# jabberjabberjabber/video-3d-pipeline

Measured on AMD Instinct MI355X. Metric: 1080p_sbs_to_4k_depth_frames_per_s, higher is better.
Workload: dtype int16 (SGM) + f64 (guided filter sums; f32 depth in/out)

## Files before the change

### video-3d-pipeline_amd/csrc/v3d_guided.hip

```cpp
#include "v3d_common.h"
#include <type_traits>

__device__ __forceinline__ double gf_rcp(double x)
{
    double r = __builtin_amdgcn_rcp(x);
    r = fma(r, fma(-x, r, 1.0), r);
    r = fma(r, fma(-x, r, 1.0), r);
    return r;
}

template <typename TD> __device__ __forceinline__ float gf_ld(const TD* p, size_t i);
template <> __device__ __forceinline__ float gf_ld<float>(const float* p, size_t i) { const float v = p[i]; return fabsf(v) <= 3.402823466e38f ? v : 0.f; }
template <> __device__ __forceinline__ float gf_ld<int16_t>(const int16_t* p, size_t i) { const int d = p[i]; return d > 0 ? (float)d * 0.0625f : 0.f; }
template <> __device__ __forceinline__ float gf_ld<uint16_t>(const uint16_t* p, size_t i) { return (float)p[i]; }

typedef unsigned short v3d_u16x2v __attribute__((ext_vector_type(2)));
typedef unsigned short v3d_u16x4 __attribute__((ext_vector_type(4)));
__device__ __forceinline__ void gf_st(float* p, float q) { *p = q; }
__device__ __forceinline__ void gf_st(uint16_t* p, float q) { *p = v3d_rint_u16(q); }

#define GF_TX 64
#define GF_RUN 8
#define GF_RMAX 16

template <typename TD>
__device__ __forceinline__ double gf_bilinear(const TD* __restrict__ src, int Ws, int Hs, double sx, double sy, int x, int y)
{
    const double fx = (x + 0.5) * sx - 0.5, fy = (y + 0.5) * sy - 0.5;
    const double x0f = floor(fx), y0f = floor(fy);
    const double wx = fx - x0f, wy = fy - y0f;
    const int x0 = (int)x0f, y0 = (int)y0f;
    const int xa = min(max(x0, 0), Ws - 1), xb = min(max(x0 + 1, 0), Ws - 1);
    const int ya = min(max(y0, 0), Hs - 1), yb = min(max(y0 + 1, 0), Hs - 1);
    const double top = (double)gf_ld(src, (size_t)ya * Ws + xa) * (1.0 - wx) + (double)gf_ld(src, (size_t)ya * Ws + xb) * wx;
    const double bot = (double)gf_ld(src, (size_t)yb * Ws + xa) * (1.0 - wx) + (double)gf_ld(src, (size_t)yb * Ws + xb) * wx;
    return top * (1.0 - wy) + bot * wy;
}

template <int SWEEP, int GF_RUNY, typename TD, typename TO>
__global__ __launch_bounds__(256) void k_gf(const TD* __restrict__ depth_lo, int Wlo, int Hlo,
                                            const uint8_t* __restrict__ guide, int W, int H, int r, double eps,
                                            double* __restrict__ A, double* __restrict__ B, TO* __restrict__ out)
{
    constexpr int NS = SWEEP == 1 ? 4 : 2;
    constexpr int GF_TY = 4 * GF_RUNY;
    extern __shared__ __attribute__((aligned(16))) double smem[];
    const int rows = GF_TY + 2 * r;
    const int pitch = (GF_TX + 2 * r) | 1;
    const int hp = GF_TX + 1;
    double* t0 = smem;
    double* t1 = t0 + rows * pitch;
    double* hs = t1 + rows * pitch;

// ... 230 lines not shown
                                asm volatile("" : "+v"(cg), "+v"(cgg) :: "memory");
                            }
                        }
                        const double s0a = cq[0] + fq[0], s0b = cq[0] + lq[0], s1a = cq[1] + fq[1], s1b = cq[1] + lq[1];
                        const int cy = min(y + RR, H - 1) - max(y - RR, 0) + 1;
                        const int cx0 = min(hgx + RR, W - 1) - max(hgx - RR, 0) + 1, cx1 = min(hgx + 1 + RR, W - 1) - max(hgx + 1 - RR, 0) + 1;
                        const double inva = gf_rcp((double)(cx0 * cy)), invb = cx1 == cx0 ? inva : gf_rcp((double)(cx1 * cy));
                        const size_t o = (size_t)y * W + hgx;
                        if (SWEEP == 1) {
                            const int sga = cg + g0, sgb = cg + gl, sgga = cgg + gg0, sggb = cgg + ggl;
                            double ab[2][2];
#pragma unroll
                            for (int n = 0; n < 2; n++) {
                                const double inv = n ? invb : inva;
                                const double mI = (double)(n ? sgb : sga) * (inv * (1.0 / 255.0)), mp = (n ? s0b : s0a) * inv;
                                const double mII = (double)(n ? sggb : sgga) * (inv * (1.0 / 65025.0)), mIp = (n ? s1b : s1a) * (inv * (1.0 / 255.0));
                                const double var = fma(-mI, mI, mII), cov = fma(-mI, mp, mIp);
                                const double a = cov * gf_rcp(var + eps);
                                ab[n][0] = a; ab[n][1] = fma(-a, mI, mp);
                            }
                            if (vec_ok) {
                                v3d_f64x2 va = { ab[0][0], ab[1][0] }, vb = { ab[0][1], ab[1][1] };
                                __builtin_nontemporal_store(va, reinterpret_cast<v3d_f64x2*>(A + o));
                                __builtin_nontemporal_store(vb, reinterpret_cast<v3d_f64x2*>(B + o));
                            } else {
                                A[o] = ab[0][0]; B[o] = ab[0][1];
                                if (px1) { A[o + 1] = ab[1][0]; B[o + 1] = ab[1][1]; }
                            }
                        } else {
                            const double Ia = (double)guide[o] * (1.0 / 255.0);
                            const double Ib = px1 ? (double)guide[o + 1] * (1.0 / 255.0) : 0.0;
                            const float qa = (float)((s0a * inva) * Ia + (s1a * inva)), qb = (float)((s0b * invb) * Ib + (s1b * invb));
                            if (vec_ok && (std::is_same<TO, float>::value || (reinterpret_cast<uintptr_t>(out + o) & 3) == 0)) {
                                if constexpr (std::is_same<TO, float>::value) {
                                    v3d_f32x2 vq = { qa, qb };
                                    __builtin_nontemporal_store(vq, reinterpret_cast<v3d_f32x2*>(out + o));
                                } else {
                                    v3d_u16x2v vq = { v3d_rint_u16(qa), v3d_rint_u16(qb) };
                                    __builtin_nontemporal_store(vq, reinterpret_cast<v3d_u16x2v*>(out + o));
                                }
                            } else {
                                gf_st(out + o, qa);
                                if (px1) gf_st(out + o + 1, qb);
                            }
                        }
                    }
                    buf ^= 1;
                }
            }
        }
    }
}

__device__ __forceinline__ int gf_swz2(int m) { return m ^ ((m >> 3) & 1) ^ ((m >> 4) & 1); }
__device__ __forceinline__ int gf_swz4(int m) { return m ^ ((m >> 4) & 3); }
__device__ __forceinline__ int gf_c8(int c) { return 2 * gf_swz2(c >> 1) + (c & 1); }

template <int RR>
__device__ __forceinline__ void gf_run4(const double* row, int c0, double s[4])
{
    const v3d_f64x2* d = reinterpret_cast<const v3d_f64x2*>(row);
    const int m0 = (c0 - RR) >> 1;
    double c = 0.0, l0 = 0.0, l1 = 0.0, l2 = 0.0, r1 = 0.0, r2 = 0.0, r3 = 0.0;
#pragma unroll
    for (int k0 = 0; k0 < RR + 2; k0 += GF_CH) {
        v3d_f64x2 w[GF_CH];
#pragma unroll
        for (int i = 0; i < GF_CH; i++) if (k0 + i < RR + 2) w[i] = d[gf_swz2(m0 + k0 + i)];
#pragma unroll
        for (int i = 0; i < GF_CH; i++) {
            const int k = k0 + i;
            if (k == 0) { l0 = w[i].x; l1 = w[i].y; c = w[i].x; c += w[i].y; }
            else if (k == 1) { l2 = w[i].x; c += w[i].x; c += w[i].y; }
            else if (k < RR) { c += w[i].x; c += w[i].y; }
            else if (k == RR) { c += w[i].x; r1 = w[i].y; }
            else if (k == RR + 1) { r2 = w[i].x; r3 = w[i].y; }
        }
        asm volatile("" : "+v"(c) :: "memory");
    }
    s[0] = c; s[1] = (s[0] + r1) - l0; s[2] = (s[1] + r2) - l1; s[3] = (s[2] + r3) - l2;
}

template <int RR>
__device__ __forceinline__ void gf_run4(const int2* row, int c0, int2 s[4])
{
    const int4* d = reinterpret_cast<const int4*>(row);
    const int m0 = (c0 - RR) >> 1;
    int2 c = make_int2(0, 0), l0 = c, l1 = c, l2 = c, r1 = c, r2 = c, r3 = c;
#pragma unroll
    for (int k0 = 0; k0 < RR + 2; k0 += 3) {
        int4 w[3];
#pragma unroll
        for (int i = 0; i < 3; i++) if (k0 + i < RR + 2) w[i] = d[gf_swz2(m0 + k0 + i)];
#pragma unroll
        for (int i = 0; i < 3; i++) {
            const int k = k0 + i;
            const int2 a = make_int2(w[i].x, w[i].y), b = make_int2(w[i].z, w[i].w);
            if (k == 0) { l0 = a; l1 = b; c = make_int2(a.x + b.x, a.y + b.y); }
            else if (k == 1) { l2 = a; c.x += a.x + b.x; c.y += a.y + b.y; }
            else if (k < RR) { c.x += a.x + b.x; c.y += a.y + b.y; }
            else if (k == RR) { c.x += a.x; c.y += a.y; r1 = b; }
            else if (k == RR + 1) { r2 = a; r3 = b; }
        }
        asm volatile("" : "+v"(c.x), "+v"(c.y) :: "memory");
    }
    s[0] = c;
    s[1] = make_int2(s[0].x + r1.x - l0.x, s[0].y + r1.y - l0.y);
    s[2] = make_int2(s[1].x + r2.x - l1.x, s[1].y + r2.y - l1.y);
    s[3] = make_int2(s[2].x + r3.x - l2.x, s[2].y + r3.y - l2.y);
}

template <int RR>
__device__ __forceinline__ void gf_run4(const int4* row, int c0, int4 s[4])
{
    int4 c = make_int4(0, 0, 0, 0), l0 = c, l1 = c, l2 = c, r1 = c, r2 = c, r3 = c;
#pragma unroll
    for (int k0 = 0; k0 < 2 * RR + 4; k0 += 3) {
        int4 u[3];
#pragma unroll
        for (int i = 0; i < 3; i++) if (k0 + i < 2 * RR + 4) u[i] = row[gf_swz4(c0 - RR + k0 + i)];
#pragma unroll
        for (int i = 0; i < 3; i++) {
            const int k = k0 + i;
            if (k < 2 * RR + 1) { c.x += u[i].x; c.y += u[i].y; c.z += u[i].z; c.w += u[i].w; }
            if (k == 0) l0 = u[i];
            else if (k == 1) l1 = u[i];
            else if (k == 2) l2 = u[i];
            else if (k == 2 * RR + 1) r1 = u[i];
            else if (k == 2 * RR + 2) r2 = u[i];
            else if (k == 2 * RR + 3) r3 = u[i];
        }
        asm volatile("" : "+v"(c.x), "+v"(c.y), "+v"(c.z), "+v"(c.w) :: "memory");
    }
    s[0] = c;
    s[1] = make_int4(s[0].x - l0.x + r1.x, s[0].y - l0.y + r1.y, s[0].z - l0.z + r1.z, s[0].w - l0.w + r1.w);
    s[2] = make_int4(s[1].x - l1.x + r2.x, s[1].y - l1.y + r2.y, s[1].z - l1.z + r2.z, s[1].w - l1.w + r2.w);
    s[3] = make_int4(s[2].x - l2.x + r3.x, s[2].y - l2.y + r3.y, s[2].z - l2.z + r3.z, s[2].w - l2.w + r3.w);
}

template <int RR>
__device__ __forceinline__ void gf_solve4(const int sg[4], const int sgg[4], const double sp[4], const double sgp[4], int hgx, int y,
                                          int W, int H, double eps, double a[4], double b[4])
{
    const int cy = min(y + RR, H - 1) - max(y - RR, 0) + 1;
    int cx[4];
#pragma unroll
    for (int n = 0; n < 4; n++) cx[n] = min(hgx + n + RR, W - 1) - max(hgx + n - RR, 0) + 1;
    const double inv0 = gf_rcp((double)(cx[0] * cy));
#pragma unroll
    for (int n = 0; n < 4; n++) {
        const double inv = (n == 0 || cx[n] == cx[0]) ? inv0 : gf_rcp((double)(cx[n] * cy));
        const double mI = (double)sg[n] * (inv * (1.0 / 255.0)), mp = sp[n] * inv;
        const double mII = (double)sgg[n] * (inv * (1.0 / 65025.0)), mIp = sgp[n] * (inv * (1.0 / 255.0));
        const double var = fma(-mI, mI, mII), cov = fma(-mI, mp, mIp);
        const double aa = cov * gf_rcp(var + eps);
        a[n] = aa; b[n] = fma(-aa, mI, mp);
    }
}

template <int RR, int COLS, typename TD, bool I1, typename TO>
__global__ __launch_bounds__(2 * COLS, I1 ? 4 : 2) void k_gff(const TD* __restrict__ depth_lo, int Wlo, int Hlo,
                                                const uint8_t* __restrict__ guide, int W, int H, double eps, int band_h,
                                                TO* __restrict__ out, size_t depth_stride, size_t guide_stride)
{
    static_assert(RR % 4 == 0, "runs of four must not straddle the strip's halo boundaries");
    static_assert(!I1 || std::is_same<TD, int16_t>::value, "the integer stage 1 takes the int16 disparity");
    static_assert(COLS == 256 || (COLS == 512 && I1), "strip width (512 columns: I1 only, the f64 route's rows exceed the LDS)");
    constexpr int R = 2 * RR + 1, NOUT = COLS - 4 * RR, HR = COLS / 4;
    constexpr int S1D = 2 * 4 * 2 * COLS * 8, S1 = I1 ? 2 * 4 * COLS * 16 : S1D + 2 * 4 * COLS * 8;
    __shared__ __attribute__((aligned(16))) unsigned char sS1[S1];
    double (*sV1)[4][2][COLS] = reinterpret_cast<double (*)[4][2][COLS]>(sS1);
    int2 (*sVi)[4][COLS] = reinterpret_cast<int2 (*)[4][COLS]>(sS1 + (I1 ? 0 : S1D));
    int4 (*sVq)[4][COLS] = reinterpret_cast<int4 (*)[4][COLS]>(sS1);
// ... 17 lines not shown
        const int gxc = min(max(gx, 0), W - 1);
        uint32_t ring[R];
        double r1[I1 ? 1 : R];
        uint32_t rgw[I1 ? 1 : (R + 3) / 4];
        int vg = 0, vgg = 0, vP = 0, vgP = 0;
        double v0 = 0.0, v1 = 0.0;
#pragma unroll
        for (int j = 0; j < R; j++) ring[j] = 0u;
#pragma unroll
        for (int j = 0; j < (I1 ? 1 : R); j++) r1[j] = 0.0;
#pragma unroll
        for (int j = 0; j < (I1 ? 1 : (R + 3) / 4); j++) rgw[j] = 0u;
        (void)ring; (void)r1; (void)rgw;
        int bxa, bxb, wxa = 0, wxb = 0; double bwx = 0.0;
        const double sx = (double)Wlo / (double)W, sy = (double)Hlo / (double)H;
        if constexpr (I1) {
            const int kx = gx >> 1;
            bxa = min(max((gx & 1) ? kx : kx - 1, 0), Wlo - 1); bxb = min(max((gx & 1) ? kx + 1 : kx, 0), Wlo - 1);
            wxa = (gx & 1) ? 3 : 1; wxb = 4 - wxa;
        } else {
            const double fx = (gx + 0.5) * sx - 0.5, x0f = floor(fx);
            bwx = fx - x0f;
            bxa = min(max((int)x0f, 0), Wlo - 1); bxb = min(max((int)x0f + 1, 0), Wlo - 1);
        }
        (void)wxa; (void)wxb; (void)bwx;
        struct RowIn { int g; typename std::conditional<I1, int, float>::type a0, a1, b0, b1; bool in; };
        auto fetch_row = [&](int tt) -> RowIn {
            RowIn q;
            const int e = ya - 2 * RR + tt;
            q.in = col_ok && e >= 0 && e < H && tt < nrows;
            const int ec = min(max(e, 0), H - 1);
            q.g = guide[(size_t)ec * W + gxc];
            if constexpr (I1) {
                const int ky = ec >> 1;
                const TD* ra = depth_lo + (size_t)min(max((ec & 1) ? ky : ky - 1, 0), Hlo - 1) * Wlo;
                const TD* rb = depth_lo + (size_t)min(max((ec & 1) ? ky + 1 : ky, 0), Hlo - 1) * Wlo;
                q.a0 = max((int)ra[bxa], 0); q.a1 = max((int)ra[bxb], 0); q.b0 = max((int)rb[bxa], 0); q.b1 = max((int)rb[bxb], 0);
            } else {
                const double fy = (e + 0.5) * sy - 0.5, y0f = floor(fy);
                const TD* ra = depth_lo + (size_t)min(max((int)y0f, 0), Hlo - 1) * Wlo;
                const TD* rb = depth_lo + (size_t)min(max((int)y0f + 1, 0), Hlo - 1) * Wlo;
                q.a0 = gf_ld(ra, bxa); q.a1 = gf_ld(ra, bxb); q.b0 = gf_ld(rb, bxa); q.b1 = gf_ld(rb, bxb);
            }
            return q;
        };
        RowIn nx[4] = { fetch_row(0), fetch_row(1), fetch_row(2), fetch_row(3) };
        for (int p0 = 0; p0 < NP; p0 += R) {
#pragma clang loop unroll(full)
            for (int sp = 0; sp < R; sp++) {
                const int p = p0 + sp;
                if (p < NP) {
                    int tl = t;
                    asm volatile("" : "+v"(tl));
                    const int hrow = tl / HR, c0 = 4 * (tl % HR), hgx = gx0 + c0;
                    const int j = p - 1;
                    if (j >= RR / 2 && j < NS) {
                        const int y = ya - 3 * RR + 4 * j + hrow;
                        double a[4] = { 0.0, 0.0, 0.0, 0.0 }, b[4] = { 0.0, 0.0, 0.0, 0.0 };
                        if (c0 >= RR && c0 < COLS - RR && y >= 0 && y < H && hgx >= 0 && hgx < W) {
                            int sg[4], sgg[4]; double sp_[4], sgp[4];
                            if constexpr (I1) {
                                int4 s[4];
                                gf_run4<RR>(&sVq[j & 1][hrow][0], c0, s);
#pragma unroll
                                for (int n = 0; n < 4; n++) {
                                    sg[n] = s[n].x; sgg[n] = s[n].y;
                                    sp_[n] = (double)s[n].z * (1.0 / 256.0); sgp[n] = (double)s[n].w * (1.0 / 256.0);
                                }
                            } else {
                                int2 si[4];
                                gf_run4<RR>(&sVi[j & 1][hrow][0], c0, si);
                                gf_run4<RR>(&sV1[j & 1][hrow][0][0], c0, sp_);
                                gf_run4<RR>(&sV1[j & 1][hrow][1][0], c0, sgp);
#pragma unroll
                                for (int n = 0; n < 4; n++) { sg[n] = si[n].x; sgg[n] = si[n].y; }
                            }
                            gf_solve4<RR>(sg, sgg, sp_, sgp, hgx, y, W, H, eps, a, b);
#pragma unroll
                            for (int n = 0; n < 4; n++) if (hgx + n >= W) { a[n] = 0.0; b[n] = 0.0; }
                        }
                        double* ab = &sAB[j % 3][hrow][0][0];
                        const int e0 = 2 * gf_swz2(c0 >> 1), e1 = 2 * gf_swz2((c0 >> 1) + 1);
                        *reinterpret_cast<v3d_f64x2*>(ab + e0) = v3d_f64x2{ a[0], a[1] };
                        *reinterpret_cast<v3d_f64x2*>(ab + e1) = v3d_f64x2{ a[2], a[3] };
                        *reinterpret_cast<v3d_f64x2*>(ab + COLS + e0) = v3d_f64x2{ b[0], b[1] };
                        *reinterpret_cast<v3d_f64x2*>(ab + COLS + e1) = v3d_f64x2{ b[2], b[3] };
                    }
                    if (p < NS) {
                        const int tA = 4 * p;
                        const RowIn cur[4] = { nx[0], nx[1], nx[2], nx[3] };
#pragma unroll
                        for (int k = 0; k < 4; k++) nx[k] = fetch_row(tA + 4 + k);
                        const bool emit = p >= RR / 2;
#pragma unroll
                        for (int rr = 0; rr < 4; rr++) {
                            const int slot = (4 * sp + rr) % R;
                            const int e = ya - 2 * RR + tA + rr;
                            if constexpr (I1) {
                                int gn = 0, Pn = 0;
                                if (cur[rr].in) {
                                    gn = cur[rr].g;
                                    const int wya = (e & 1) ? 3 : 1;
                                    Pn = wya * (wxa * cur[rr].a0 + wxb * cur[rr].a1) + (4 - wya) * (wxa * cur[rr].b0 + wxb * cur[rr].b1);
                                }
                                const int go = (int)(ring[slot] & 0xFFu), Po = (int)(ring[slot] >> 8);
                                ring[slot] = ((uint32_t)Pn << 8) | (uint32_t)gn;
                                vg += gn - go; vgg += gn * gn - go * go;
                                vP += Pn - Po; vgP += gn * Pn - go * Po;
                                if (emit) sVq[p & 1][rr][gf_swz4(t)] = make_int4(vg, vgg, vP, vgP);
                            } else {
                                int gn = 0; double pn = 0.0;
                                if (cur[rr].in) {
                                    gn = cur[rr].g;
                                    const double fy = (e + 0.5) * sy - 0.5, wy = fy - floor(fy);
                                    const double a0 = (double)cur[rr].a0, b0 = (double)cur[rr].b0;
                                    const double top = fma(bwx, (double)cur[rr].a1 - a0, a0);
                                    const double bot = fma(bwx, (double)cur[rr].b1 - b0, b0);
                                    pn = fma(wy, bot - top, top);
                                }
                                const int go = (int)((rgw[slot >> 2] >> (8 * (slot & 3))) & 0xFFu); const double po = r1[slot];
                                rgw[slot >> 2] = (rgw[slot >> 2] & ~(0xFFu << (8 * (slot & 3)))) | ((uint32_t)gn << (8 * (slot & 3)));
                                r1[slot] = pn;
                                vg += gn - go; vgg += gn * gn - go * go;
                                v0 += pn - po; v1 = fma((double)gn, pn, fma(-(double)go, po, v1));
                                if (emit) {
                                    const int ct = gf_c8(t);
                                    sV1[p & 1][rr][0][ct] = v0; sV1[p & 1][rr][1][ct] = v1;
                                    sVi[p & 1][rr][ct] = make_int2(vg, vgg);
                                }
                            }
                        }
                    }
                    __syncthreads();
                }
            }
        }
    } else {
        double r0[R], r1[R], va = 0.0, vb = 0.0;
#pragma unroll
        for (int j = 0; j < R; j++) { r0[j] = 0.0; r1[j] = 0.0; }
        for (int p0 = 0; p0 < NP; p0 += R) {
#pragma clang loop unroll(full)
            for (int sp = 0; sp < R; sp++) {
                const int p = p0 + sp;
                if (p < NP) {
                    int tl = t;
                    asm volatile("" : "+v"(tl));
                    const int hrow = tl / HR, c0 = 4 * (tl % HR), hgx = gx0 + c0;
                    {
                        const int j = p - 3;
                        const int y = ya - 4 * RR + 4 * j + hrow;
                        if (j >= RR && j < NS && c0 >= 2 * RR && c0 < COLS - 2 * RR && hgx < W && y < yb) {
                            double sa[4], sb[4];
                            gf_run4<RR>(&sAB[j % 3][hrow][0][0], c0, sa);
                            gf_run4<RR>(&sAB[j % 3][hrow][1][0], c0, sb);
                            const int cy = min(y + RR, H - 1) - max(y - RR, 0) + 1;
                            int cx[4];
#pragma unroll
                            for (int n = 0; n < 4; n++) cx[n] = min(hgx + n + RR, W - 1) - max(hgx + n - RR, 0) + 1;
                            const double inv0 = gf_rcp((double)(cx[0] * cy));
                            const size_t o = (size_t)y * W + hgx;
                            const bool all_in = hgx + 3 < W;
                            const bool vec_ok = all_in && (W & 3) == 0 && ((reinterpret_cast<uintptr_t>(out + o) | reinterpret_cast<uintptr_t>(guide + o)) & 3) == 0
                                                && (reinterpret_cast<uintptr_t>(out + o) & (4 * sizeof(TO) - 1)) == 0;
                            int g[4];
                            if (vec_ok) {
                                const uint32_t g4 = *reinterpret_cast<const uint32_t*>(guide + o);
#pragma unroll
                                for (int n = 0; n < 4; n++) g[n] = (g4 >> (8 * n)) & 0xFF;
                            } else {
#pragma unroll
                                for (int n = 0; n < 4; n++) g[n] = hgx + n < W ? guide[o + n] : 0;
                            }
                            float q[4];
#pragma unroll
                            for (int n = 0; n < 4; n++) {
                                const double inv = (n == 0 || cx[n] == cx[0]) ? inv0 : gf_rcp((double)(cx[n] * cy));
                                const double I = (double)g[n] * (1.0 / 255.0);
                                q[n] = (float)((sa[n] * inv) * I + (sb[n] * inv));
                            }
                            if (vec_ok) {
                                if constexpr (std::is_same<TO, float>::value) {
                                    const v3d_f32x4 vq = { q[0], q[1], q[2], q[3] };
                                    __builtin_nontemporal_store(vq, reinterpret_cast<v3d_f32x4*>(out + o));
                                } else {
                                    const v3d_u16x4 vq = { v3d_rint_u16(q[0]), v3d_rint_u16(q[1]), v3d_rint_u16(q[2]), v3d_rint_u16(q[3]) };
                                    __builtin_nontemporal_store(vq, reinterpret_cast<v3d_u16x4*>(out + o));
                                }
                            } else {
#pragma unroll
                                for (int n = 0; n < 4; n++) if (hgx + n < W) gf_st(out + o + n, q[n]);
                            }
                        }
                    }
                    {
                        const int j = p - 2;
                        if (j >= RR / 2 && j < NS) {
                            const bool emit = j >= RR;
                            double* col = &sAB[j % 3][0][0][gf_c8(tl)];
#pragma unroll
                            for (int rr = 0; rr < 4; rr++) {
                                const int slot = (4 * sp + rr) % R;
                                const double n0 = col[rr * 2 * COLS], n1 = col[rr * 2 * COLS + COLS];
                                const double o0 = r0[slot], o1 = r1[slot];
                                r0[slot] = n0; r1[slot] = n1;
                                va += n0 - o0; vb += n1 - o1;
                                if (emit) { col[rr * 2 * COLS] = va; col[rr * 2 * COLS + COLS] = vb; }
                            }
                        }
                    }
                    __syncthreads();
                }
            }
        }
    }
}

template <int RR, typename TD, typename TO>
static void launch_gff(const TD* depth_lo, int Wlo, int Hlo, const uint8_t* guide, int W, int H, double eps,
                       TO* out, int n, size_t depth_stride, size_t guide_stride, hipStream_t st)
{
    bool i1 = false;
    if constexpr (std::is_same<TD, int16_t>::value) i1 = g_v3d_opt.gf_int1 && W == 2 * Wlo && H == 2 * Hlo;
    const int cols = g_v3d_opt.gf_cols == 512 && i1 ? 512 : 256;
    int band = g_v3d_opt.gf_band;
    if (band <= 0) {
        int dev = 0, ncu = 256;
        (void)hipGetDevice(&dev);
        (void)hipDeviceGetAttribute(&ncu, hipDeviceAttributeMultiprocessorCount, dev);
        const long slots = (long)ncu * (cols == 256 && i1 ? 2 : 1), strips = v3d_cdiv(W, cols - 4 * RR);
        long best = -1;
        for (int nb = 1; nb <= 64 && nb <= H; nb++) {
            const int b = (v3d_cdiv(H, nb) + 1) & ~1;
            const long wgs = strips * v3d_cdiv(H, b) * n, rounds = (wgs + slots - 1) / slots, cost = rounds * (b + 4 * RR);
            if (best < 0 || cost < best) { best = cost; band = b; }
        }
    }
    const dim3 grid(v3d_cdiv(W, cols - 4 * RR), v3d_cdiv(H, band), n);
    if constexpr (std::is_same<TD, int16_t>::value) {
        if (i1 && cols == 512) {
            hipLaunchKernelGGL((k_gff<RR, 512, TD, true, TO>), grid, dim3(1024), 0, st, depth_lo, Wlo, Hlo, guide, W, H, eps, band, out, depth_stride, guide_stride);
            return;
        }
        if (i1) {
            hipLaunchKernelGGL((k_gff<RR, 256, TD, true, TO>), grid, dim3(512), 0, st, depth_lo, Wlo, Hlo, guide, W, H, eps, band, out, depth_stride, guide_stride);
            return;
        }
    }
    hipLaunchKernelGGL((k_gff<RR, 256, TD, false, TO>), grid, dim3(512), 0, st, depth_lo, Wlo, Hlo, guide, W, H, eps, band, out, depth_stride, guide_stride);
}

template <int RR, typename TD, typename TO>
// ... 93 lines not shown
```

### video-3d-pipeline_amd/csrc/v3d_sgbm_cost.hip

```cpp
#include "v3d_sgbm_internal.h"

#ifndef PF_BAND
#define PF_BAND 64
#endif
__global__ __launch_bounds__(256) void k_prefilter(const uint8_t* __restrict__ img1, const uint8_t* __restrict__ img2,
                                                   int W, int H, int pitch, size_t frame_stride, int ft,
                                                   uint4* __restrict__ rec)
{
    __shared__ uint8_t sI[2][2][256];
    __shared__ unsigned short sGR[2][2][256];
    const int t = threadIdx.x, f = blockIdx.z;
    const int x = blockIdx.x * 252 - 2 + t;
    const int xc = min(max(x, 0), W - 1);
    const bool xin = x > 0 && x < W - 1;
    const int ya = blockIdx.y * PF_BAND, yb = min(ya + PF_BAND, H);
    const uint8_t* I0 = img1 + f * frame_stride + xc;
    const uint8_t* I1 = img2 + f * frame_stride + xc;
    auto ld = [&](int y) -> uint32_t {
        const size_t o = (size_t)min(max(y, 0), H - 1) * pitch;
        return (uint32_t)I0[o] | ((uint32_t)I1[o] << 8);
    };
    int dm[2], d0[2], r0[2];
    {
        const uint32_t vm = ld(ya - 1), v0 = ld(ya);
// ... 8 lines not shown
            r0[im] = (v0 >> (8 * im)) & 0xFF;
        }
        __syncthreads();
    }
    uint32_t nxt = ld(ya + 1);
    int gp[2] = { 0, 0 }, rp[2] = { 0, 0 };
    const int tl = max(t - 1, 0), tr = min(t + 1, 255);
    for (int y = ya; y <= yb; y++) {
        const int par = y & 1;
        const uint32_t ve = nxt;
        nxt = ld(y + 2);
        sI[par][0][t] = (uint8_t)ve; sI[par][1][t] = (uint8_t)(ve >> 8);
        sGR[par][0][t] = (unsigned short)(gp[0] | (rp[0] << 8));
        sGR[par][1][t] = (unsigned short)(gp[1] | (rp[1] << 8));
        __syncthreads();
        uint32_t out[4];
#pragma unroll
        for (int im = 0; im < 2; im++) {
            const int g = gp[im], r = rp[im];
            const int lo = sGR[par][im][tl], hi = sGR[par][im][tr];
            int gl = g, gr = g, rl = r, rr = r;
            if (x > 0) { gl = (g + (lo & 0xFF)) >> 1; rl = (r + (lo >> 8)) >> 1; }
            if (x < W - 1) { gr = (g + (hi & 0xFF)) >> 1; rr = (r + (hi >> 8)) >> 1; }
            const int g0 = min(min(gl, gr), g), g1 = max(max(gl, gr), g);
            const int q0 = min(min(rl, rr), r), q1 = max(max(rl, rr), r);
            out[2 * im] = (uint32_t)g | ((uint32_t)g0 << 8) | ((uint32_t)g1 << 16);
            out[2 * im + 1] = (uint32_t)r | ((uint32_t)q0 << 8) | ((uint32_t)q1 << 16);
            const int de = (int)sI[par][im][tr] - (int)sI[par][im][tl];
            const int dup = y > 0 ? dm[im] : d0[im];
            const int ddn = y < H - 1 ? de : d0[im];
            gp[im] = xin ? min(max(2 * d0[im] + dup + ddn, -ft), ft) + ft : ft;
            rp[im] = xin ? r0[im] : ft;
            dm[im] = d0[im]; d0[im] = de; r0[im] = (ve >> (8 * im)) & 0xFF;
        }
        if (y > ya && t >= 2 && t <= 253 && x < W)
            st_stream(rec + ((size_t)f * H + (y - 1)) * W + x, make_uint4(out[0], out[1], out[2], out[3]));
    }
}

template <int LPC> struct CostGeo {
    static constexpr int EP = 64 / LPC, NP = EP / 2, COLS = 512 / LPC, OUT = COLS - 4, NREC = COLS + 64;
};
#ifndef V3D_COST_LPC
#define V3D_COST_LPC 8
#endif

__device__ __forceinline__ uint32_t bt_pair(uint32_t U, uint32_t U0, uint32_t U1, uint32_t V, uint32_t V0, uint32_t V1)
{
    const uint32_t a = pk_max(pk_subu_sat(U, V1), pk_subu_sat(V0, U));
    const uint32_t b = pk_max(pk_subu_sat(V, U1), pk_subu_sat(U0, V));
    return pk_min(a, b);
}

#ifndef V3D_COST_WAVES
#define V3D_COST_WAVES 6
#endif
template <int LPC>
__global__ __launch_bounds__(512, V3D_COST_WAVES) void k_cost(const uint4* __restrict__ rec,
                                              int W, int H, int W1, int lofs, int band_h, int P2, unsigned char* __restrict__ C, int xcd_order)
{
    typedef CostGeo<LPC> G;
    constexpr int EP = G::EP, NP = G::NP, COLS = G::COLS, OUT = G::OUT, NREC = G::NREC;
    typedef typename VecT<EP>::type vec_t;
    constexpr int RROW = (NREC + 4) / 2, RCOPY = 6 * RROW + (LPC == 8 ? 3 : 0), RBUF = 2 * RCOPY;
    __shared__ __attribute__((aligned(8))) uint32_t sRV[2 * RBUF];
    __shared__ __attribute__((aligned(8))) uint32_t sUL[2][COLS][6];
    __shared__ vec_t sPix[2][COLS][LPC];

    const int tid = threadIdx.x, col = tid / LPC, dq = tid % LPC;
    int bxi = blockIdx.x, byi = blockIdx.y, bzi = blockIdx.z;
    if (xcd_order) xcd_tile(bxi, byi, bzi);
    const int xr0 = bxi * OUT;
    const int ys = byi * band_h, ye = min(ys + band_h, H);
    const int f = bzi;
    const uint32_t* rf = reinterpret_cast<const uint32_t*>(rec + (size_t)f * H * W);
    unsigned char* Cf = C + (size_t)f * c_frame(H, W1);
    static_assert(LPC == 8, "the store packs a lane's 8 disparities into one 12-byte field");

    const int xrc = min(max(xr0 - 2 + col, 0), W1 - 1);
    const int k0 = NREC - 66 - (xrc - xr0) + EP * dq;
    const int rcopy = k0 & 1, rk = k0 - rcopy;
    const int rv_off = rcopy * RCOPY + rk / 2;
    const bool out_col = (col >= 2) && (col < 2 + OUT) && (xr0 - 2 + col < W1);
    const int hc = min(max(col, 2), COLS - 3);
    const int nrows = (ye - ys) + 4;

    const int half = tid & 1, ri = tid >> 1, lt = (tid - 256) >> 1;
    const bool ld_right = ri < NREC, ld_left = tid >= 256 && lt < COLS;
    uint32_t ld_a = 0, ld_b = 0;
    int st_off = 0;
    if (ld_right) {
        ld_a = 4 * min(max(xr0 - 1 + ri, 0), W - 1) + 2 + half;
        ld_b = 4 * min(max(xr0 - 2 + ri, 0), W - 1) + 2 + half;
        const int k = NREC - 1 - ri;
        st_off = (k & 1) * RCOPY + 3 * half * RROW + (k >> 1);
    } else if (ld_left) {
        ld_a = ld_b = 4 * (min(max(xr0 - 2 + lt, 0), W1 - 1) + lofs) + half;
        st_off = lt * 6 + 3 * half;
    }
    const bool ld_any = ld_right || ld_left;
    auto stage = [&](int b, uint2 rec) {
        if (ld_right) {
#pragma unroll
            for (int j = 0; j < 3; j++)
                sRV[b * RBUF + st_off + j * RROW] = __builtin_amdgcn_perm(rec.y, rec.x, 0x0c000c00u | (uint32_t)j | ((uint32_t)(4 + j) << 16));
        } else if (ld_left) {
#pragma unroll
            for (int j = 0; j < 3; j++)
                (&sUL[b][0][0])[st_off + j] = __builtin_amdgcn_perm(rec.x, rec.x, 0x0c000c00u | (uint32_t)j | ((uint32_t)j << 16));
        }
    };
    const __amdgpu_buffer_rsrc_t rs_rec = buf_rsrc(rf, (uint32_t)H * W * 16u), rs_c = buf_rsrc(Cf, (uint32_t)c_frame(H, W1));
    const uint32_t la = ld_any ? ld_a * 4u : V3D_BUF_OOB, lb = ld_any ? ld_b * 4u : V3D_BUF_OOB;
    auto fetch = [&](int k) -> uint2 {
        const uint32_t ro = (uint32_t)min(max(ys - 2 + min(k, nrows - 1), 0), H - 1) * W * 16u;
        return make_uint2(buf_load_u32(rs_rec, ro + la), buf_load_u32(rs_rec, ro + lb));
    };
    if (ld_any) stage(0, fetch(0));
    uint2 nr[2];
    nr[1] = fetch(1); nr[0] = fetch(2);
    __syncthreads();

    uint32_t ring[5][NP], vs[NP];
#pragma unroll
    for (int j = 0; j < NP; j++) { vs[j] = 0u;
#pragma unroll
        for (int i = 0; i < 5; i++) ring[i][j] = 0u; }
    const uint32_t st_col = out_col ? (uint32_t)((xr0 - 2 + col) * C_PXB + c_lane_off<EP>(dq)) : V3D_BUF_OOB;

    for (int k10 = 0; k10 < nrows; k10 += 10) {
#pragma unroll
      for (int s10 = 0; s10 < 10; s10++) {
        const int k = k10 + s10;
        if (k >= nrows) break;
        const int slot = s10 % 5, buf = s10 & 1;

        uint32_t pix[NP];
#pragma unroll
        for (int pl = 0; pl < 2; pl++) {
            uint32_t U[3], V[3][NP];
#pragma unroll
            for (int i = 0; i < 3; i++) {
                U[i] = sUL[buf][col][3 * pl + i];
                const uint32_t* pr = &sRV[buf * RBUF + rv_off + (3 * pl + i) * RROW];
#pragma unroll
                for (int j = 0; j < NP; j++) V[i][j] = pr[j];
            }
#pragma unroll
            for (int j = 0; j < NP; j++) {
                const uint32_t c = bt_pair(U[0], U[1], U[2], V[0][j], V[1][j], V[2][j]);
                pix[j] = pl == 0 ? c : pix[j] + pk_shr_u(c, 2);
            }
            if (pl == 0) { if (NP == 4) asm volatile("" : "+v"(pix[0]), "+v"(pix[1]), "+v"(pix[NP - 2]), "+v"(pix[NP - 1]) :: "memory");
                           else asm volatile("" : "+v"(pix[0]), "+v"(pix[NP - 1]) :: "memory"); }
        }
        sPix[buf][col][dq] = Packer<NP>::go(pix);

        if (k + 1 < nrows && ld_any) stage(buf ^ 1, nr[buf ^ 1]);
        nr[buf ^ 1] = fetch(k + 3);
        __syncthreads();

        {
            uint32_t h[NP], w[NP];
            vec_unpack<NP>(sPix[buf][hc - 2][dq], h);
#pragma unroll
            for (int t = -1; t <= 2; t++) {
                vec_unpack<NP>(sPix[buf][hc + t][dq], w);
#pragma unroll
                for (int j = 0; j < NP; j++) h[j] += w[j];
            }
#pragma unroll
            for (int j = 0; j < NP; j++) { vs[j] += h[j] - ring[slot][j]; ring[slot][j] = h[j]; }
            const uint32_t st_row = k >= 4 ? (uint32_t)c_row(ys + k - 4, W1) : V3D_BUF_OOB;
            const uint32_t st_off = __builtin_elementwise_add_sat(st_col, st_row);
            {
                uint32_t t[NP];
#pragma unroll
                for (int j = 0; j < NP; j++)
                    asm("v_bfi_b32 %0, %1, %2, %3" : "=v"(t[j]) : "s"(0xFFFu), "v"(vs[j]), "v"(vs[j] >> 4));
                const v3d_u32x3_a4 pk = { __builtin_amdgcn_perm(t[1], t[0], 0x04020100u), __builtin_amdgcn_perm(t[2], t[1], 0x05040201u),
                                          __builtin_amdgcn_perm(t[NP - 1], t[2], 0x06050402u) };
                __builtin_amdgcn_raw_buffer_store_b96(pk, rs_c, st_off, 0, 2);
            }
        }
      }
    }
}

__global__ __launch_bounds__(256) void k_c_export(const unsigned char* __restrict__ C, size_t npx, int P2, int16_t* __restrict__ out)
{
    const size_t i = (size_t)blockIdx.x * 256 + threadIdx.x, px = i >> 3;
    const int dl = (int)(i & 7);
    if (px >= npx) return;
    const uint4 v = c_unpack(*reinterpret_cast<const typename CRaw<8>::type*>(C + px * C_PXB + c_lane_off<8>(dl)), dl, pk_bcast(P2));
    *reinterpret_cast<uint4*>(out + px * V3D_D + 8 * dl) = v;
}

int sgbm_cost_volume(v3d_sgbm* h, const uint8_t* left, const uint8_t* right, int n, int W, int H, int pitch, size_t frame_stride, hipStream_t st)
{
    const int W1 = W - V3D_D;
    prof_mark(h, ST_PREFILTER, st);
    hipLaunchKernelGGL(k_prefilter, dim3(v3d_cdiv(W, 252), v3d_cdiv(H, PF_BAND), n), dim3(256), 0, st, left, right, W, H, pitch, frame_stride, h->ftzero, h->rec);
    prof_mark(h, ST_COST, st);
    constexpr int COST_OUT = CostGeo<V3D_COST_LPC>::OUT;
    hipLaunchKernelGGL((k_cost<V3D_COST_LPC>), dim3(v3d_cdiv(W1, COST_OUT), v3d_cdiv(H, h->cost_band), n), dim3(512), 0, st, h->rec, W, H, W1, V3D_D + h->prm.minDisparity, h->cost_band, h->P2, h->C, h->cost_xcd);
    V3D_LAUNCH_CHECK();
    return V3D_OK;
}

int sgbm_export_cost(const v3d_sgbm* h, int W, int H, int16_t* C_out, hipStream_t st)
{
    const size_t npx = (size_t)(W - V3D_D) * H;
    hipLaunchKernelGGL(k_c_export, dim3((unsigned)((npx * 8 + 255) / 256)), dim3(256), 0, st, h->C, npx, h->P2, C_out);
    V3D_LAUNCH_CHECK();
    return V3D_OK;
}
```

Measured before the change: 2588.

## Replace XOR-swizzled shared-memory layout with parity-interleaved layout in guided filter

Replaces the XOR swizzles (gf_swz2/gf_swz4/gf_c8) on the guided-filter shared-memory row buffers with a layout that splits columns by parity or by mod 4 into separate contiguous sections. Each horizontal running-sum load then becomes a per-thread base pointer plus a compile-time constant offset, which removes per-load swizzle arithmetic. The layout is meant to keep consecutive threads on distinct LDS banks. The vertical pass now indexes by the raw thread id, relying on that pass being elementwise and in place. The new layout could bring back bank conflicts if the interleave maps threads poorly, and it depends on COLS being divisible by 4.

```diff
diff --git a/video-3d-pipeline_amd/csrc/v3d_gf_layout.h b/video-3d-pipeline_amd/csrc/v3d_gf_layout.h
--- /dev/null
+++ b/video-3d-pipeline_amd/csrc/v3d_gf_layout.h
@@ -0,0 +1,16 @@
+#pragma once
+
+#if defined(__HIPCC__)
+#define GF_LAY_FN __host__ __device__ __forceinline__ constexpr
+#else
+#define GF_LAY_FN static inline
+#endif
+
+GF_LAY_FN int gf_pair_chunk(int m, int cols) { return (m & 1) * (cols / 4) + (m >> 1); }
+GF_LAY_FN int gf_pair_elem(int c, int cols) { return 2 * gf_pair_chunk(c >> 1, cols) + (c & 1); }
+GF_LAY_FN int gf_pair_col(int t, int cols) { return t < cols / 2 ? (4 * (t >> 1) | (t & 1)) : (4 * ((t - cols / 2) >> 1) | 2 | (t & 1)); }
+GF_LAY_FN int gf_run_base(int u, int r) { return u - r / 4; }
+GF_LAY_FN int gf_pair_run_off(int k, int cols) { return (k & 1) * (cols / 4) + (k >> 1); }
+
+GF_LAY_FN int gf_quad_slot(int c, int cols) { return (c & 3) * (cols / 4) + (c >> 2); }
+GF_LAY_FN int gf_quad_run_off(int k, int cols) { return (k & 3) * (cols / 4) + (k >> 2); }
diff --git a/video-3d-pipeline_amd/csrc/v3d_guided.hip b/video-3d-pipeline_amd/csrc/v3d_guided.hip
--- a/video-3d-pipeline_amd/csrc/v3d_guided.hip
+++ b/video-3d-pipeline_amd/csrc/v3d_guided.hip
@@ -1,4 +1,5 @@
 #include "v3d_common.h"
+#include "v3d_gf_layout.h"
 #include <type_traits>
 
 __device__ __forceinline__ double gf_rcp(double x)
@@ -335,21 +336,16 @@
     }
 }
 
-__device__ __forceinline__ int gf_swz2(int m) { return m ^ ((m >> 3) & 1) ^ ((m >> 4) & 1); }
-__device__ __forceinline__ int gf_swz4(int m) { return m ^ ((m >> 4) & 3); }
-__device__ __forceinline__ int gf_c8(int c) { return 2 * gf_swz2(c >> 1) + (c & 1); }
-
-template <int RR>
-__device__ __forceinline__ void gf_run4(const double* row, int c0, double s[4])
-{
-    const v3d_f64x2* d = reinterpret_cast<const v3d_f64x2*>(row);
-    const int m0 = (c0 - RR) >> 1;
+template <int RR, int COLS>
+__device__ __forceinline__ void gf_run4(const double* row, int u, double s[4])
+{
+    const v3d_f64x2* d = reinterpret_cast<const v3d_f64x2*>(row) + gf_run_base(u, RR);
     double c = 0.0, l0 = 0.0, l1 = 0.0, l2 = 0.0, r1 = 0.0, r2 = 0.0, r3 = 0.0;
 #pragma unroll
     for (int k0 = 0; k0 < RR + 2; k0 += GF_CH) {
         v3d_f64x2 w[GF_CH];
 #pragma unroll
-        for (int i = 0; i < GF_CH; i++) if (k0 + i < RR + 2) w[i] = d[gf_swz2(m0 + k0 + i)];
+        for (int i = 0; i < GF_CH; i++) if (k0 + i < RR + 2) w[i] = d[gf_pair_run_off(k0 + i, COLS)];
 #pragma unroll
         for (int i = 0; i < GF_CH; i++) {
             const int k = k0 + i;
@@ -364,17 +360,16 @@
     s[0] = c; s[1] = (s[0] + r1) - l0; s[2] = (s[1] + r2) - l1; s[3] = (s[2] + r3) - l2;
 }
 
-template <int RR>
-__device__ __forceinline__ void gf_run4(const int2* row, int c0, int2 s[4])
-{
-    const int4* d = reinterpret_cast<const int4*>(row);
-    const int m0 = (c0 - RR) >> 1;
+template <int RR, int COLS>
+__device__ __forceinline__ void gf_run4(const int2* row, int u, int2 s[4])
+{
+    const int4* d = reinterpret_cast<const int4*>(row) + gf_run_base(u, RR);
     int2 c = make_int2(0, 0), l0 = c, l1 = c, l2 = c, r1 = c, r2 = c, r3 = c;
 #pragma unroll
     for (int k0 = 0; k0 < RR + 2; k0 += 3) {
         int4 w[3];
 #pragma unroll
-        for (int i = 0; i < 3; i++) if (k0 + i < RR + 2) w[i] = d[gf_swz2(m0 + k0 + i)];
+        for (int i = 0; i < 3; i++) if (k0 + i < RR + 2) w[i] = d[gf_pair_run_off(k0 + i, COLS)];
 #pragma unroll
         for (int i = 0; i < 3; i++) {
             const int k = k0 + i;
@@ -393,15 +388,16 @@
     s[3] = make_int2(s[2].x + r3.x - l2.x, s[2].y + r3.y - l2.y);
 }
 
-template <int RR>
-__device__ __forceinline__ void gf_run4(const int4* row, int c0, int4 s[4])
-{
-    int4 c = make_int4(0, 0, 0, 0), l0 = c, l1 = c, l2 = c, r1 = c, r2 = c, r3 = c;
+template <int RR, int COLS>
+__device__ __forceinline__ void gf_run4(const int4* row, int u, int4 s[4])
+{
+    const int4* d = row + gf_run_base(u, RR);
+    int4 c =make_int4(0, 0, 0, 0), l0 = c, l1 = c, l2 = c, r1 = c, r2 = c, r3 = c;
 #pragma unroll
     for (int k0 = 0; k0 < 2 * RR + 4; k0 += 3) {
         int4 u[3];
 #pragma unroll
-        for (int i = 0; i < 3; i++) if (k0 + i < 2 * RR + 4) u[i] = row[gf_swz4(c0 - RR + k0 + i)];
+        for (int i = 0; i < 3; i++) if (k0 + i < 2 * RR + 4) u[i] = d[gf_quad_run_off(k0 + i, COLS)];
 #pragma unroll
         for (int i = 0; i < 3; i++) {
             const int k = k0 + i;
@@ -525,7 +521,7 @@
                 if (p < NP) {
                     int tl = t;
                     asm volatile("" : "+v"(tl));
-                    const int hrow = tl / HR, c0 = 4 * (tl % HR), hgx = gx0 + c0;
+                    const int hrow = tl / HR, hu = tl % HR, c0 = 4 * hu, hgx = gx0 + c0;
                     const int j = p - 1;
                     if (j >= RR / 2 && j < NS) {
                         const int y = ya - 3 * RR + 4 * j + hrow;
@@ -534,7 +530,7 @@
                             int sg[4], sgg[4]; double sp_[4], sgp[4];
                             if constexpr (I1) {
                                 int4 s[4];
-                                gf_run4<RR>(&sVq[j & 1][hrow][0], c0, s);
+                                gf_run4<RR, COLS>(&sVq[j & 1][hrow][0], hu, s);
 #pragma unroll
                                 for (int n = 0; n < 4; n++) {
                                     sg[n] = s[n].x; sgg[n] = s[n].y;
@@ -542,9 +538,9 @@
                                 }
                             } else {
                                 int2 si[4];
-                                gf_run4<RR>(&sVi[j & 1][hrow][0], c0, si);
-                                gf_run4<RR>(&sV1[j & 1][hrow][0][0], c0, sp_);
-                                gf_run4<RR>(&sV1[j & 1][hrow][1][0], c0, sgp);
+                                gf_run4<RR, COLS>(&sVi[j & 1][hrow][0], hu, si);
+                                gf_run4<RR, COLS>(&sV1[j & 1][hrow][0][0], hu, sp_);
+                                gf_run4<RR, COLS>(&sV1[j & 1][hrow][1][0], hu, sgp);
 #pragma unroll
                                 for (int n = 0; n < 4; n++) { sg[n] = si[n].x; sgg[n] = si[n].y; }
                             }
@@ -553,7 +549,7 @@
                             for (int n = 0; n < 4; n++) if (hgx + n >= W) { a[n] = 0.0; b[n] = 0.0; }
                         }
                         double* ab = &sAB[j % 3][hrow][0][0];
-                        const int e0 = 2 * gf_swz2(c0 >> 1), e1 = 2 * gf_swz2((c0 >> 1) + 1);
+                        const int e0 = 2 * gf_pair_chunk(2 * hu, COLS), e1 = 2 * gf_pair_chunk(2 * hu + 1, COLS);
                         *reinterpret_cast<v3d_f64x2*>(ab + e0) = v3d_f64x2{ a[0], a[1] };
                         *reinterpret_cast<v3d_f64x2*>(ab + e1) = v3d_f64x2{ a[2], a[3] };
                         *reinterpret_cast<v3d_f64x2*>(ab + COLS + e0) = v3d_f64x2{ b[0], b[1] };
@@ -580,7 +576,7 @@
                                 ring[slot] = ((uint32_t)Pn << 8) | (uint32_t)gn;
                                 vg += gn - go; vgg += gn * gn - go * go;
                                 vP += Pn - Po; vgP += gn * Pn - go * Po;
-                                if (emit) sVq[p & 1][rr][gf_swz4(t)] = make_int4(vg, vgg, vP, vgP);
+                                if (emit) sVq[p & 1][rr][gf_quad_slot(t, COLS)] = make_int4(vg, vgg, vP, vgP);
                             } else {
                                 int gn = 0; double pn = 0.0;
                                 if (cur[rr].in) {
@@ -597,7 +593,7 @@
                                 vg += gn - go; vgg += gn * gn - go * go;
                                 v0 += pn - po; v1 = fma((double)gn, pn, fma(-(double)go, po, v1));
                                 if (emit) {
-                                    const int ct = gf_c8(t);
+                                    const int ct = gf_pair_elem(t, COLS);
                                     sV1[p & 1][rr][0][ct] = v0; sV1[p & 1][rr][1][ct] = v1;
                                     sVi[p & 1][rr][ct] = make_int2(vg, vgg);
                                 }
@@ -619,14 +615,14 @@
                 if (p < NP) {
                     int tl = t;
                     asm volatile("" : "+v"(tl));
-                    const int hrow = tl / HR, c0 = 4 * (tl % HR), hgx = gx0 + c0;
+                    const int hrow = tl / HR, hu = tl % HR, c0 = 4 * hu, hgx = gx0 + c0;
                     {
                         const int j = p - 3;
                         const int y = ya - 4 * RR + 4 * j + hrow;
                         if (j >= RR && j < NS && c0 >= 2 * RR && c0 < COLS - 2 * RR && hgx < W && y < yb) {
                             double sa[4], sb[4];
-                            gf_run4<RR>(&sAB[j % 3][hrow][0][0], c0, sa);
-                            gf_run4<RR>(&sAB[j % 3][hrow][1][0], c0, sb);
+                            gf_run4<RR, COLS>(&sAB[j % 3][hrow][0][0], hu, sa);
+                            gf_run4<RR, COLS>(&sAB[j % 3][hrow][1][0], hu, sb);
                             const int cy = min(y + RR, H - 1) - max(y - RR, 0) + 1;
                             int cx[4];
 #pragma unroll
@@ -670,7 +666,7 @@
                         const int j = p - 2;
                         if (j >= RR / 2 && j < NS) {
                             const bool emit = j >= RR;
-                            double* col = &sAB[j % 3][0][0][gf_c8(tl)];
+                            double* col = &sAB[j % 3][0][0][tl];
 #pragma unroll
                             for (int rr = 0; rr < 4; rr++) {
                                 const int slot = (4 * sp + rr) % R;
```

After: 2615 (median of 6 runs). +1.0%, better.

## Remap cost kernel threads to column-per-lane with DPP box sums and LDS transpose

Applied to the files above, without the earlier changes.

Threads are remapped so each wave covers 64 consecutive columns for one disparity group. The horizontal 5-tap box sum now uses DPP row shifts inside the wave instead of an LDS round-trip through sPix. Right-image samples are staged into four LDS copies at staggered offsets so each lane can use aligned 8-byte reads without bank conflicts. Packed results are transposed through a swizzled LDS buffer so global stores stay coalesced per pixel. The cost is doubled LDS stores when staging and extra LDS for the transpose; DPP row shifts do not cross 16-lane rows, which could affect edge columns.

```diff
diff --git a/video-3d-pipeline_amd/csrc/v3d_sgbm_cost.hip b/video-3d-pipeline_amd/csrc/v3d_sgbm_cost.hip
--- a/video-3d-pipeline_amd/csrc/v3d_sgbm_cost.hip
+++ b/video-3d-pipeline_amd/csrc/v3d_sgbm_cost.hip
@@ -84,6 +84,14 @@
     return pk_min(a, b);
 }
 
+__device__ __forceinline__ uint32_t wave_shr1(uint32_t v) { return (uint32_t)__builtin_amdgcn_update_dpp(0, (int)v, 0x138, 0xF, 0xF, true); }
+typedef uint32_t v3d_u32x3_a16 __attribute__((ext_vector_type(3), aligned(16)));
+typedef uint32_t v3d_u32x4_a16 __attribute__((ext_vector_type(4)));
+typedef __attribute__((address_space(3))) v3d_u32x4_a16 v3d_lds_u32x4;
+typedef uint32_t v3d_u32x2_a8 __attribute__((ext_vector_type(2)));
+typedef __attribute__((address_space(3))) v3d_u32x2_a8 v3d_lds_u32x2;
+constexpr int rb_next(int lo, int res, int m = 64) { return lo + ((res - lo) % m + m) % m; }
+
 #ifndef V3D_COST_WAVES
 #define V3D_COST_WAVES 6
 #endif
@@ -93,13 +101,16 @@
 {
     typedef CostGeo<LPC> G;
     constexpr int EP = G::EP, NP = G::NP, COLS = G::COLS, OUT = G::OUT, NREC = G::NREC;
-    typedef typename VecT<EP>::type vec_t;
-    constexpr int RROW = (NREC + 4) / 2, RCOPY = 6 * RROW + (LPC == 8 ? 3 : 0), RBUF = 2 * RCOPY;
-    __shared__ __attribute__((aligned(8))) uint32_t sRV[2 * RBUF];
-    __shared__ __attribute__((aligned(8))) uint32_t sUL[2][COLS][6];
-    __shared__ vec_t sPix[2][COLS][LPC];
-
-    const int tid = threadIdx.x, col = tid / LPC, dq = tid % LPC;
+    constexpr int RROW = (NREC + 4) / 2, RQ = 6 * RROW;
+    constexpr int RB0 = 0, RB3 = rb_next(RB0 + RQ, RB0 + 17), RB2 = rb_next(RB3 + RQ, RB0 + 33), RB1 = rb_next(RB2 + RQ, RB0 + 50);
+    constexpr int RBUF = (RB1 + RQ + 1) & ~1;
+    static_assert(RROW % 2 == 0 && RB0 % 2 == 0 && RB1 % 2 == 0 && RB2 % 2 == 1 && RB3 % 2 == 1, "8-byte aligned reads");
+    static_assert((RB0 / 2 + 1) % 32 == 1 && ((RB3 + 1) / 2) % 32 == 9 && ((RB2 + 1) / 2) % 32 == 17 && (RB1 / 2) % 32 == 25, "the four copies' runs of 8 pair slots tile the 32");
+    __shared__ __attribute__((aligned(16))) uint32_t sRV[2 * RBUF];
+    __shared__ __attribute__((aligned(16))) uint32_t sUL[2][COLS][6];
+    __shared__ uint4 sX[2][COLS][8];
+
+    const int tid = threadIdx.x, col = tid & 63, dq = __builtin_amdgcn_readfirstlane(tid >> 6);
     int bxi = blockIdx.x, byi = blockIdx.y, bzi = blockIdx.z;
     if (xcd_order) xcd_tile(bxi, byi, bzi);
     const int xr0 = bxi * OUT;
@@ -111,21 +122,23 @@
 
     const int xrc = min(max(xr0 - 2 + col, 0), W1 - 1);
     const int k0 = NREC - 66 - (xrc - xr0) + EP * dq;
-    const int rcopy = k0 & 1, rk = k0 - rcopy;
-    const int rv_off = rcopy * RCOPY + rk / 2;
-    const bool out_col = (col >= 2) && (col < 2 + OUT) && (xr0 - 2 + col < W1);
-    const int hc = min(max(col, 2), COLS - 3);
+    const int rcopy = k0 & 3;
+    const int rv_base = rcopy == 0 ? RB0 : rcopy == 1 ? RB1 : rcopy == 2 ? RB2 : RB3;
+    const int rv_off = rv_base + (k0 >> 1);
+    const int xl = tid >> 3, xf = tid & 7;
+    const bool out_col = (xl >= 4) && (xr0 + xl - 4 < W1);
     const int nrows = (ye - ys) + 4;
 
     const int half = tid & 1, ri = tid >> 1, lt = (tid - 256) >> 1;
     const bool ld_right = ri < NREC, ld_left = tid >= 256 && lt < COLS;
     uint32_t ld_a = 0, ld_b = 0;
-    int st_off = 0;
+    int st_off = 0, st_twin = 0;
     if (ld_right) {
         ld_a = 4 * min(max(xr0 - 1 + ri, 0), W - 1) + 2 + half;
         ld_b = 4 * min(max(xr0 - 2 + ri, 0), W - 1) + 2 + half;
         const int k = NREC - 1 - ri;
-        st_off = (k & 1) * RCOPY + 3 * half * RROW + (k >> 1);
+        st_off = ((k & 1) ? RB1 : RB0) + 3 * half * RROW + (k >> 1);
+        st_twin = (k & 1) ? RB3 - RB1 : RB2 - RB0;
     } else if (ld_left) {
         ld_a = ld_b = 4 * (min(max(xr0 - 2 + lt, 0), W1 - 1) + lofs) + half;
         st_off = lt * 6 + 3 * half;
@@ -134,8 +147,11 @@
     auto stage = [&](int b, uint2 rec) {
         if (ld_right) {
 #pragma unroll
-            for (int j = 0; j < 3; j++)
-                sRV[b * RBUF + st_off + j * RROW] = __builtin_amdgcn_perm(rec.y, rec.x, 0x0c000c00u | (uint32_t)j | ((uint32_t)(4 + j) << 16));
+            for (int j = 0; j < 3; j++) {
+                const uint32_t v = __builtin_amdgcn_perm(rec.y, rec.x, 0x0c000c00u | (uint32_t)j | ((uint32_t)(4 + j) << 16));
+                sRV[b * RBUF + st_off + j * RROW] = v;
+                sRV[b * RBUF + st_off + st_twin + j * RROW] = v;
+            }
         } else if (ld_left) {
 #pragma unroll
             for (int j = 0; j < 3; j++)
@@ -144,8 +160,10 @@
     };
     const __amdgpu_buffer_rsrc_t rs_rec = buf_rsrc(rf, (uint32_t)H * W * 16u), rs_c = buf_rsrc(Cf, (uint32_t)c_frame(H, W1));
     const uint32_t la = ld_any ? ld_a * 4u : V3D_BUF_OOB, lb = ld_any ? ld_b * 4u : V3D_BUF_OOB;
+    const int h_last = __builtin_amdgcn_readfirstlane(H - 1);
+    const uint32_t row_bytes = (uint32_t)__builtin_amdgcn_readfirstlane(W * 16);
     auto fetch = [&](int k) -> uint2 {
-        const uint32_t ro = (uint32_t)min(max(ys - 2 + min(k, nrows - 1), 0), H - 1) * W * 16u;
+        const uint32_t ro = (uint32_t)min(max(ys - 2 + min(k, nrows - 1), 0), h_last) * row_bytes;
         return make_uint2(buf_load_u32(rs_rec, ro + la), buf_load_u32(rs_rec, ro + lb));
     };
     if (ld_any) stage(0, fetch(0));
@@ -158,7 +176,7 @@
     for (int j = 0; j < NP; j++) { vs[j] = 0u;
 #pragma unroll
         for (int i = 0; i < 5; i++) ring[i][j] = 0u; }
-    const uint32_t st_col = out_col ? (uint32_t)((xr0 - 2 + col) * C_PXB + c_lane_off<EP>(dq)) : V3D_BUF_OOB;
+    const uint32_t st_col = out_col ? (uint32_t)((xr0 + xl - 4) * C_PXB + c_lane_off<EP>(xf)) : V3D_BUF_OOB;
 
     for (int k10 = 0; k10 < nrows; k10 += 10) {
 #pragma unroll
@@ -168,15 +186,19 @@
         const int slot = s10 % 5, buf = s10 & 1;
 
         uint32_t pix[NP];
+        const volatile v3d_lds_u32x2* rv2 = (const volatile v3d_lds_u32x2*)sRV + buf * (RBUF / 2) + rv_off / 2;
+        const volatile v3d_lds_u32x2* ul2 = (const volatile v3d_lds_u32x2*)&sUL[buf][col][0];
+        const v3d_u32x2_a8 ug0 = ul2[0], ug1 = ul2[1];
 #pragma unroll
         for (int pl = 0; pl < 2; pl++) {
             uint32_t U[3], V[3][NP];
+            if (pl == 0) { U[0] = ug0.x; U[1] = ug0.y; U[2] = ug1.x; }
+            else { const v3d_u32x2_a8 ur = ul2[2]; U[0] = ug1.y; U[1] = ur.x; U[2] = ur.y; }
 #pragma unroll
             for (int i = 0; i < 3; i++) {
-                U[i] = sUL[buf][col][3 * pl + i];
-                const uint32_t* pr = &sRV[buf * RBUF + rv_off + (3 * pl + i) * RROW];
-#pragma unroll
-                for (int j = 0; j < NP; j++) V[i][j] = pr[j];
+                static_assert(NP == 4, "a lane's 8 elements are two aligned 8-byte reads");
+                const v3d_u32x2_a8 lo = rv2[(3 * pl + i) * (RROW / 2)], hi = rv2[(3 * pl + i) * (RROW / 2) + 1];
+                V[i][0] = lo.x; V[i][1] = lo.y; V[i][2] = hi.x; V[i][3] = hi.y;
             }
 #pragma unroll
             for (int j = 0; j < NP; j++) {
@@ -186,34 +208,36 @@
             if (pl == 0) { if (NP == 4) asm volatile("" : "+v"(pix[0]), "+v"(pix[1]), "+v"(pix[NP - 2]), "+v"(pix[NP - 1]) :: "memory");
                            else asm volatile("" : "+v"(pix[0]), "+v"(pix[NP - 1]) :: "memory"); }
         }
-        sPix[buf][col][dq] = Packer<NP>::go(pix);
-
+
+        {
+            uint32_t h[NP];
+#pragma unroll
+            for (int j = 0; j < NP; j++) h[j] = pix[j];
+#pragma unroll
+            for (int t = 0; t < 4; t++)
+#pragma unroll
+                for (int j = 0; j < NP; j++) h[j] = pix[j] + wave_shr1(h[j]);
+#pragma unroll
+            for (int j = 0; j < NP; j++) { vs[j] += h[j] - ring[slot][j]; ring[slot][j] = h[j]; }
+            {
+                uint32_t t[NP];
+#pragma unroll
+                for (int j = 0; j < NP; j++)
+                    asm("v_bfi_b32 %0, %1, %2, %3" : "=v"(t[j]) : "s"(0xFFFu), "v"(vs[j]), "v"(vs[j] >> 4));
+                const v3d_u32x3_a16 pk = { __builtin_amdgcn_perm(t[1], t[0], 0x04020100u), __builtin_amdgcn_perm(t[2], t[1], 0x05040201u),
+                                           __builtin_amdgcn_perm(t[NP - 1], t[2], 0x06050402u) };
+                *reinterpret_cast<v3d_u32x3_a16*>(&sX[buf][col][dq ^ (col & 7)]) = pk;
+            }
+        }
         if (k + 1 < nrows && ld_any) stage(buf ^ 1, nr[buf ^ 1]);
         nr[buf ^ 1] = fetch(k + 3);
         __syncthreads();
-
         {
-            uint32_t h[NP], w[NP];
-            vec_unpack<NP>(sPix[buf][hc - 2][dq], h);
-#pragma unroll
-            for (int t = -1; t <= 2; t++) {
-                vec_unpack<NP>(sPix[buf][hc + t][dq], w);
-#pragma unroll
-                for (int j = 0; j < NP; j++) h[j] += w[j];
-            }
-#pragma unroll
-            for (int j = 0; j < NP; j++) { vs[j] += h[j] - ring[slot][j]; ring[slot][j] = h[j]; }
             const uint32_t st_row = k >= 4 ? (uint32_t)c_row(ys + k - 4, W1) : V3D_BUF_OOB;
             const uint32_t st_off = __builtin_elementwise_add_sat(st_col, st_row);
-            {
-                uint32_t t[NP];
-#pragma unroll
-                for (int j = 0; j < NP; j++)
-                    asm("v_bfi_b32 %0, %1, %2, %3" : "=v"(t[j]) : "s"(0xFFFu), "v"(vs[j]), "v"(vs[j] >> 4));
-                const v3d_u32x3_a4 pk = { __builtin_amdgcn_perm(t[1], t[0], 0x04020100u), __builtin_amdgcn_perm(t[2], t[1], 0x05040201u),
-                                          __builtin_amdgcn_perm(t[NP - 1], t[2], 0x06050402u) };
-                __builtin_amdgcn_raw_buffer_store_b96(pk, rs_c, st_off, 0, 2);
-            }
+            const v3d_u32x4_a16 x = *(const volatile v3d_lds_u32x4*)&sX[buf][xl][xf ^ (xl & 7)];
+            const v3d_u32x3_a4 pk = { x.x, x.y, x.z };
+            __builtin_amdgcn_raw_buffer_store_b96(pk, rs_c, st_off, 0, 2);
         }
       }
     }
```

Result: no change. 2593 before, 2615 after, median of 6 (+0.9%).
